# nh273/caro-ai

Hardware: NVIDIA B200
Metric: connect4_mcts_leaf_evals_per_sec (higher is better)
Workload: dtype f16

## Files before the change

caro-ai_b200/csrc/net.cu:

```cuda
#include <cuda_runtime.h>
#include <math.h>

#include <atomic>

#include "../../include/caro_b200.h"
#include "common_host.h"
#include "net.h"
#include "rules.cuh"

namespace caro {

__device__ __forceinline__ float lrelu(float x) { return x > 0.0f ? x : kLeaky * x; }

template <class R, int F>
__global__ void __launch_bounds__(256)
net_simt_kernel(R rules, const typename R::Board* __restrict__ boards, const uint8_t* __restrict__ who,
                const int32_t* __restrict__ d_count, long long max_count, const float* __restrict__ blob, BlobLayout L,
                int A, float* __restrict__ probs, float* __restrict__ values) {
  extern __shared__ float sm[];
  const int H = rules.rows(), W = rules.cols(), HW = H * W;
  const long long count = d_count ? min((long long)*d_count, max_count) : max_count;
  float* buf0 = sm;
  float* buf1 = sm + F * HW;
  for (long long leaf = blockIdx.x; leaf < count; leaf += gridDim.x) {
// ... 139 lines not shown
  if (ce != cudaSuccess) return caro_fail(CARO_E_CUDA, cudaGetErrorString(ce));
  if (net->layout.filters == kWideFilters) return caro_net_wide_pack(net, h_blob);
  const int rc = caro_net_tc_pack(net, h_blob);
  if (rc != CARO_OK) return rc;
  if (!caro_net_rt_supports(net)) return CARO_OK;
  const int rc2 = caro_net_rt_pack(net, h_blob);
  return rc2 != CARO_OK ? rc2 : caro_net_rx_pack(net, h_blob);
}

static int net_create(int rows, int cols, int actions, const BlobLayout& layout, const float* h_blob, size_t n_floats, caro_net** out) {
  static std::atomic<unsigned long long> next_serial{0};
  caro_net* net = new caro_net();
  net->serial = ++next_serial;
  net->version = 0;
  net->H = rows;
  net->W = cols;
  net->A = actions;
  net->layout = layout;
  net->d_blob = nullptr;
  net->d_tc_weights = nullptr;
  net->d_rt_weights = nullptr;
  net->d_rt_pair_weights = nullptr;
  net->d_rt_f16_weights = nullptr;
  net->d_tc_pair_weights = nullptr;
  net->d_rt_scratch = nullptr;
  net->rt_scratch_seq = 0;
  net->d_rx_weights = nullptr;
  net->d_wide_weights = nullptr;
  net->d_tc_bias = nullptr;
  net->d_pol_fc_t = nullptr;
  net->d_trace = nullptr;
  net->d_headfeat = nullptr;
  net->d_heads_b = nullptr;
  net->headfeat_leaves = 0;
  net->headfeat_seq = 0;
  net->grid_limit = 0;
  net->pipeline_limit = 0;
  {
    int dev = 0;
    cudaGetDevice(&dev);
    net->sm_count = 148;
    cudaDeviceGetAttribute(&net->sm_count, cudaDevAttrMultiProcessorCount, dev);
    int prc = caro_net_tc_prepare();
    if (prc == CARO_OK) prc = caro_net_rt_prepare();
    if (prc == CARO_OK) prc = caro_net_rx_prepare();
    if (prc == CARO_OK) prc = caro_net_heads_prepare();
// ... 113 lines not shown
```

caro-ai_b200/csrc/net.h:

```cpp
#pragma once
#include <cuda_runtime.h>
#include <stddef.h>
#include <stdint.h>

namespace caro {

constexpr int kFilters = 64;
constexpr int kWideFilters = 128;
constexpr int kBlocks = 5;
constexpr int kMaxBlocks = 20;
constexpr float kLeaky = 0.01f;

struct BlobLayout {
  size_t conv_in_w, conv_in_b;
  size_t conv_w[kMaxBlocks], conv_b[kMaxBlocks];
  int blocks;
  int filters;
  size_t val_conv_w, val_conv_b, val_fc1_w, val_fc1_b, val_fc2_w, val_fc2_b;
  size_t pol_conv_w, pol_conv_b, pol_fc_w, pol_fc_b;
  size_t total;
};

inline BlobLayout blob_layout(int H, int W, int A, int blocks = kBlocks, int filters = kFilters) {
  BlobLayout L;
// ... 15 lines not shown
  L.val_fc1_w = take(20 * hw);
  L.val_fc1_b = take(20);
  L.val_fc2_w = take(20);
  L.val_fc2_b = take(1);
  L.pol_conv_w = take(2 * F);
  L.pol_conv_b = take(2);
  L.pol_fc_w = take((size_t)A * 2 * hw);
  L.pol_fc_b = take(A);
  L.total = o;
  return L;
}

}

struct caro_net {
  int H, W, A;
  caro::BlobLayout layout;
  float* d_blob;
  void* d_tc_weights;
  void* d_rt_weights;
  void* d_tc_pair_weights;
  void* d_rt_f16_weights;
  void* d_rt_pair_weights;
  void* d_rt_scratch;
  unsigned rt_scratch_seq;
  void* d_rx_weights;
  void* d_wide_weights;
  alignas(16) float h_rt_consts[(caro::kMaxBlocks + 1) * 64 + 3 * 64 + 4 + 1536 + 4];
  float* d_tc_bias;
  float* d_pol_fc_t;
  void* d_headfeat;
  void* d_heads_b;
  long long headfeat_leaves;
  unsigned headfeat_seq;
  void* d_trace;
  int sm_count;
  int grid_limit;
  unsigned long long serial;
  unsigned long long version;
  int pipeline_limit;
};

void caro_pipeline_forget(unsigned long long engine_serial, unsigned long long net_serial);

int caro_net_tc_pack(caro_net* net, const float* h_blob);
int caro_net_tc_prepare();
// ... 31 lines not shown
```

caro-ai_b200/csrc/net_rt.cu:

```cuda
#include <cuda_bf16.h>
#include <cuda_fp16.h>
#include <cuda_fp8.h>
#include <cuda_runtime.h>
#include <math.h>
#include <string.h>

#include <type_traits>
#include <vector>

#include "../../include/caro_b200.h"
#include "common_host.h"
#include "net.h"
#include "rules.cuh"

#include "tc_common.cuh"
#include "rt_common.cuh"

#ifndef CARO_RT_MAXREG
#define CARO_RT_MAXREG 96
#endif
#ifndef CARO_RT_CP
#define CARO_RT_CP 2
#endif

namespace caro {

template <int CP, bool PAIR_ = false, bool F16_ = false>
struct RtCfg {
  static constexpr bool kPair = PAIR_;
  static constexpr bool kF16 = F16_;
  static_assert(!(PAIR_ && F16_), "the pair form exists for the bf16 mode only");
  static constexpr int kBlockBytes = PAIR_ ? kRtPairBlockBytes : kRtBlockBytes;
  static constexpr int kBlockUnits = kBlockBytes / 16;
  static constexpr int kRegionBytes = kRtRegionBlocks * kBlockBytes;
  static constexpr int kCP = CP;
  static constexpr int kCH = 64 / CP;
  static constexpr int kEpiWarps = 4 * CP;
  static constexpr int kEpiThreads = kEpiWarps * 32;
  static constexpr int kMmaWarp = kEpiWarps;
  static constexpr int kLoadWarp = kEpiWarps + 1;
  static constexpr int kHeadWarp = kEpiWarps + 2;
  static constexpr int kHeadWarps = 4;
  static constexpr int kHeadThreads = 32 * kHeadWarps;
  static constexpr int kThreads = kEpiThreads + 64 + kHeadThreads;
  static_assert(CP == 2 || CP == 4, "two or four channel parts");
  static_assert(CP == 2 || !PAIR_, "the pair form is built for two channel parts");
  static constexpr int kAct = 0;
  static constexpr int kWgt = kAct + kRtActBytes;
  static constexpr int kHeadF = kWgt + kRtRegions * kRegionBytes;
  static constexpr int kFc = kHeadF + (PAIR_ ? 0 : kRtHeadFloats * 4);
  static constexpr int kFcW = kFc + (PAIR_ ? 0 : kRtFcFloats * 4);
  static constexpr int kBars0 = kFcW;
  static constexpr int kNumBars = kRtRegions * kRtRegionBlocks + 2 * kRtRegions + 2 * kRtMaxH + 2;
  static constexpr int kFixed = kBars0 + kNumBars * 8 + 32;
// ... 43 lines not shown
                            (POS == 0 ? (uint64_t)kRtPairTop : POS == 2 ? (uint64_t)kRtPairBottom : 0ull);
        umma_bf16_pair(d_main, ad, bd, POS == 1 ? rt_idesc_pair(192) : rt_idesc_pair(128), 1u);
        if (POS == 2 && (i == 5 || i == NB - 1)) umma_commit_pair_a(i < 6 ? empty0 : empty1);
      } else {
        const uint64_t bd = (i < 6 ? rb0 + (uint64_t)(i * kUnits) : rb1 + (uint64_t)((i - 6) * kUnits)) + (POS == 0 ? 64ull : 0ull);
        if (POS == 1 && i == 0) {
          umma_bf16(d_main, ad, bd, rt_idesc_fmt<F16>(128), 1u);
          umma_bf16(d_new, ad, bd + 128ull, rt_idesc_fmt<F16>(64), 0u);
        } else {
          umma_bf16(d_main, ad, bd, POS == 1 ? rt_idesc_fmt<F16>(192) : rt_idesc_fmt<F16>(128), (POS == 0 && i == 0) ? 0u : 1u);
        }
        if (POS == 2 && (i == 5 || i == NB - 1)) umma_commit_a(i < 6 ? empty0 : empty1);
      }
    }
  }
}

template <class R, class K, int HC>
__global__ void __maxnreg__(CARO_RT_MAXREG)
net_rt_kernel(R rules, RtGeom gm, const typename R::Board* __restrict__ boards, const uint8_t* __restrict__ who,
              const int32_t* __restrict__ d_count, long long max_count, const uint8_t* __restrict__ wimg,
              const __grid_constant__ RtConsts consts, const float* __restrict__ blob, BlobLayout L,
              const float* __restrict__ pol_fc_t, const float* __restrict__ val_fc1_t, float* __restrict__ probs,
              float* __restrict__ values, long long* __restrict__ trace, float* __restrict__ scratch) {
  constexpr bool PAIR = K::kPair;
  extern __shared__ __align__(128) uint8_t smem[];
  uint8_t* act = smem + K::kAct;
  uint8_t* wgt = smem + K::kWgt;
  float* headf_s = PAIR ? scratch + (size_t)blockIdx.x * (kRtHeadFloats + kRtFcFloats) : reinterpret_cast<float*>(smem + K::kHeadF);
  float* fc_s = PAIR ? headf_s + kRtHeadFloats : reinterpret_cast<float*>(smem + K::kFc);
  uint64_t* bar_full = reinterpret_cast<uint64_t*>(smem + K::kBars);
  uint64_t* bar_empty = bar_full + kRtRegions * kRtRegionBlocks;
  uint64_t* bar_fullp = bar_empty + kRtRegions;
  uint64_t* bar_acc = bar_fullp + kRtRegions;
  uint64_t* bar_act = bar_acc + kRtMaxH;
  uint64_t* bar_feat = bar_act + kRtMaxH;
  uint32_t* tmem_slot = reinterpret_cast<uint32_t*>(bar_feat + 2);

  const int tid = threadIdx.x;
  const int warp = tid >> 5;
  if (tid == 0) TC_TRACE(7, 0);
  long long* gt_slot = nullptr;
  if (trace != nullptr && tid == 0 && (blockIdx.x == 0 || blockIdx.x == gridDim.x - 1) && trace[7998] == 2) {
    long long* base = trace + 8000 + (blockIdx.x == 0 ? 0 : 4096);
    const long long k = base[0];
    base[0] = k + 1;
    if (k < 2040) {
      gt_slot = base + 1 + 2 * k;
// ... 67 lines not shown
    }
    asm volatile("bar.sync 2, %0;" ::"n"(K::kHeadThreads) : "memory");
    for (int gi = 0; gi + 1 < my_groups; ++gi) {
      const long long leaf0 = group_leaf0(gi);
      const int nvalid = group_valid(leaf0);
      mbar_wait_relaxed(bar_feat + 0, (uint32_t)gi & 1u);
      rt_heads<K::kHeadThreads, 2>(gm, nvalid, leaf0, htid, headf_s, fc_s, consts.headb[0], consts.headb[1], consts.headb[2], fcv, polw,
                                   valw, probs, values, consts);
      mbar_arrive(bar_feat + 1);
      if (htid == 0) TC_TRACE(5, gi);
    }
    {
      const int gi = my_groups - 1;
      const long long leaf0 = group_leaf0(gi);
      const int nvalid = group_valid(leaf0);
      mbar_wait(bar_feat + 0, (uint32_t)gi & 1u);
      rt_heads<K::kEpiThreads + K::kHeadThreads, 3>(gm, nvalid, leaf0, K::kEpiThreads + htid, headf_s, fc_s, consts.headb[0],
                                                    consts.headb[1], consts.headb[2], fcv, polw, valw, probs, values, consts);
      if (htid == 0) TC_TRACE(5, gi);
    }
  } else if (warp == K::kLoadWarp) {
    if ((tid & 31) == 0) {
      const int regions_net = 2 * gm.layers - 1;
      const int total = my_groups * regions_net;
      const uint8_t* wrank = wimg + (size_t)rank * regions_net * K::kRegionBytes;
      int reg = 0, src = 0;
      uint32_t round = 0;
      for (int n = 0; n < total; ++n) {
        if (round > 0) mbar_wait_relaxed(bar_empty + reg, (round - 1u) & 1u);
        const int nblk = src == 0 ? 3 : kRtRegionBlocks;
        uint64_t* bar = bar_full + reg * kRtRegionBlocks;
        mbar_expect_tx(bar, (uint32_t)(nblk * K::kBlockBytes));
        for (int b = 0; b < nblk; ++b)
          bulk_g2s(wgt + (reg * kRtRegionBlocks + b) * K::kBlockBytes, wrank + (size_t)(src * kRtRegionBlocks + b) * K::kBlockBytes,
                   (uint32_t)K::kBlockBytes, bar);
        if (++reg == kRtRegions) { reg = 0; ++round; }
        if (++src == regions_net) src = 0;
      }
    }
  } else if (warp == K::kMmaWarp && PAIR && rank != 0) {
    if ((tid & 31) == 0) {
      const int total = my_groups * (2 * gm.layers - 1);
      const uint32_t fullp_leader = mapa_a(smem_u32(bar_fullp), 0u);
      int reg = 0;
      uint32_t ph = 0;
      for (int n = 0; n < total; ++n) {
        mbar_wait(bar_full + reg * kRtRegionBlocks, ph);
        mbar_arrive_cluster_a(fullp_leader + 8u * (uint32_t)reg);
        if (++reg == kRtRegions) { reg = 0; ph ^= 1u; }
      }
    }
  } else if (warp == K::kMmaWarp) {
    uint32_t elected;
    asm volatile("{\n\t.reg .pred P;\n\telect.sync _|P, 0xffffffff;\n\tselp.u32 %0, 1, 0, P;\n\t}" : "=r"(elected));
    const uint64_t a_desc0 = make_desc(smem_u32(act) + (uint32_t)kRtHalo * 16u, (uint32_t)kRtChunkBytes, 128u);
    const uint64_t b_desc0 = make_desc(smem_u32(wgt), (PAIR ? (uint32_t)kRtPairRows : 192u) * 16u, 128u);
    uint32_t full_a = smem_u32(bar_full), empty_a = smem_u32(bar_empty), acc_a = smem_u32(bar_acc), act_a = smem_u32(bar_act);
    uint32_t fullp_a = smem_u32(bar_fullp);
    asm volatile("" : "+r"(full_a), "+r"(empty_a), "+r"(acc_a), "+r"(act_a), "+r"(fullp_a));
    const bool tr = elected && trace != nullptr && blockIdx.x == 0;
#define RT_MMA_TRACE(kind, idx)                                                 \
  do {                                                                          \
    if (tr && (idx) < 1000) trace[(kind) * 1000 + (idx)] = clock64();           \
  } while (0)
    const int n_layers = gm.layers;
    const int total_layers = my_groups * n_layers;
    int reg = 0;
    uint32_t rphase = 0;
    int layer = 0;
    bool pre_waited = false;
    struct LayerW {
      uint64_t rb0, rb1;
      uint32_t full0, full1, empty0, empty1, ph0, ph1, fullp0, fullp1;
    };
    auto take_regions = [&](bool first_l) {
      LayerW w;
      w.rb0 = b_desc0 + (uint64_t)(uint32_t)(reg * kRtRegionBlocks * K::kBlockUnits);
      w.full0 = full_a + 8u * (uint32_t)(reg * kRtRegionBlocks);
      w.empty0 = empty_a + 8u * (uint32_t)reg;
      w.fullp0 = fullp_a + 8u * (uint32_t)reg;
      w.ph0 = rphase;
      if (++reg == kRtRegions) { reg = 0; rphase ^= 1u; }
      w.rb1 = w.rb0;
      w.full1 = w.full0;
      w.empty1 = w.empty0;
      w.fullp1 = w.fullp0;
      w.ph1 = w.ph0;
      if (!first_l) {
        w.rb1 = b_desc0 + (uint64_t)(uint32_t)(reg * kRtRegionBlocks * K::kBlockUnits);
        w.full1 = full_a + 8u * (uint32_t)(reg * kRtRegionBlocks);
        w.empty1 = empty_a + 8u * (uint32_t)reg;
        w.fullp1 = fullp_a + 8u * (uint32_t)reg;
        w.ph1 = rphase;
        if (++reg == kRtRegions) { reg = 0; rphase ^= 1u; }
      }
      return w;
    };
    LayerW nxt = take_regions(true);
    for (int gl = 0; gl < total_layers; ++gl) {
      const uint32_t par = (uint32_t)gl & 1u;
      RT_MMA_TRACE(6, gl * 2);
      const bool first = layer == 0;
      const LayerW cur = nxt;
      const uint64_t rb0 = cur.rb0, rb1 = cur.rb1;
      const uint32_t full0 = cur.full0, full1 = cur.full1, empty0 = cur.empty0, empty1 = cur.empty1, ph0 = cur.ph0, ph1 = cur.ph1;
      const uint32_t fullp0 = cur.fullp0, fullp1 = cur.fullp1;
      auto mid = [&]() {
        nxt = take_regions(layer + 1 == n_layers);
        asm volatile("" : "+l"(nxt.rb0), "+l"(nxt.rb1), "+r"(nxt.full0), "+r"(nxt.full1), "+r"(nxt.empty0), "+r"(nxt.empty1), "+r"(nxt.ph0),
                     "+r"(nxt.ph1));
        if (PAIR) asm volatile("" : "+r"(nxt.fullp0), "+r"(nxt.fullp1));
      };
      auto tile = [&](auto yv) {
        const int y = rt_value(yv);
        if (y == 0 && !pre_waited) {
          if (PAIR) {
            mbar_wait_cluster_a(act_a, par);
            mbar_wait_cluster_a(act_a + 8u, par);
          } else {
            mbar_wait_a(act_a, par);
            mbar_wait_a(act_a + 8u, par);
          }
        }
        if (y == 0) RT_MMA_TRACE(6, gl * 2 + 1);
        tc_fence_after();
        RT_MMA_TRACE(0, gl * 8 + y);
        const uint64_t a_tile = a_desc0 + (uint64_t)(uint32_t)(y * 128);
        uint64_t rb0t = rb0, rb1t = rb1;
        asm volatile("" : "+l"(rb0t), "+l"(rb1t));
        const uint32_t d_main = tmem_base + (uint32_t)(y == 0 ? 0 : (y - 1) * 64);
        const uint32_t d_new = tmem_base + (uint32_t)((y + 1) * 64);
        uint32_t nb0 = 0u, nb1 = 0u;
        uint32_t npar = par;
        if (y + 2 < H) {
          nb0 = act_a + 8u * (uint32_t)(y + 2);
        } else if (y == H - 1 && H >= 4 && gl + 1 < total_layers) {
          nb0 = act_a;
          nb1 = act_a + 8u;
          npar = par ^ 1u;
        }
        if (first) {
          if (y == 0) rt_issue_tile<0, true, PAIR, K::kF16>(y == 1, mid, elected, a_tile, rb0t, rb1t, d_main, d_new, full0, full1, ph0, ph1, empty0, empty1, nb0, nb1, npar, fullp0, fullp1);
          else if (y == H - 1) rt_issue_tile<2, true, PAIR, K::kF16>(y == 1, mid, elected, a_tile, rb0t, rb1t, d_main, d_new, full0, full1, ph0, ph1, empty0, empty1, nb0, nb1, npar, fullp0, fullp1);
          else rt_issue_tile<1, true, PAIR, K::kF16>(y == 1, mid, elected, a_tile, rb0t, rb1t, d_main, d_new, full0, full1, ph0, ph1, empty0, empty1, nb0, nb1, npar, fullp0, fullp1);
        } else {
          if (y == 0) rt_issue_tile<0, false, PAIR, K::kF16>(y == 1, mid, elected, a_tile, rb0t, rb1t, d_main, d_new, full0, full1, ph0, ph1, empty0, empty1, nb0, nb1, npar, fullp0, fullp1, tr && gl < 100 ? trace + 5000 + gl * 6 : nullptr);
          else if (y == H - 1) rt_issue_tile<2, false, PAIR, K::kF16>(y == 1, mid, elected, a_tile, rb0t, rb1t, d_main, d_new, full0, full1, ph0, ph1, empty0, empty1, nb0, nb1, npar, fullp0, fullp1);
          else rt_issue_tile<1, false, PAIR, K::kF16>(y == 1, mid, elected, a_tile, rb0t, rb1t, d_main, d_new, full0, full1, ph0, ph1, empty0, empty1, nb0, nb1, npar, fullp0, fullp1);
        }
        if (elected) {
          if (PAIR) umma_commit_pair_a(acc_a + 8u * (uint32_t)y);
          else umma_commit_a(acc_a + 8u * (uint32_t)y);
        }
        RT_MMA_TRACE(1, gl * 8 + y);
        __syncwarp();
      };
      if constexpr (HC == 6) {
        tile(RtInt<0>{});
        tile(RtInt<1>{});
        tile(RtInt<2>{});
        tile(RtInt<3>{});
        tile(RtInt<4>{});
        tile(RtInt<5>{});
      } else {
#pragma unroll 1
        for (int y = 0; y < H; ++y) tile(y);
      }
      pre_waited = H >= 4 && gl + 1 < total_layers;
      if (++layer == n_layers) layer = 0;
    }
#undef RT_MMA_TRACE
  } else {
    const int quarter = warp & 3, cp = warp >> 2;
    constexpr int CH = K::kCH, QN = CH / 4, C8N = CH / 8;
    const int row = quarter * 32 + (tid & 31);
    const int bidx = row >> gm.pshift, col = row & (gm.pitch - 1);
    const bool real = col < gm.W;
    const uint32_t lane_base = (uint32_t)(quarter * 32) << 16;
    const int HW = gm.H * gm.W;
    const bool dbg_skip_epilogue = trace != nullptr && trace[7999] == 1;
    const uint32_t act_leader = PAIR ? mapa_a(smem_u32(bar_act), 0u) : 0u;
    auto act_arrive = [&](int y) {
      if (PAIR) {
        __syncwarp();
        if ((tid & 31) == 0) mbar_arrive_cluster_a(act_leader + 8u * (uint32_t)y);
      } else {
        mbar_arrive(bar_act + y);
      }
    };
    const bool dbg_no_zero = trace != nullptr && (trace[7996] & 1);
    auto zero_acc = [&](int y, int c0) {
      if (dbg_no_zero) return;
      const uint32_t a = tmem_base + lane_base + (uint32_t)(y * 64 + c0);
      TMEM_ST16Z(a, 0u);
      TMEM_ST16Z(a + 16u, 0u);
    };

    auto write_inputs = [&](int y, long long leaf0, int writer) {
      if (cp == writer) {
        uint32_t lo = 0u;
        const long long leaf = leaf0 + bidx;
        if (real && leaf < count) {
          const typename R::Board s = boards[leaf];
          const int wm = who[leaf];
          constexpr uint32_t kOne = K::kF16 ? 0x3C00u : 0x3F80u;
          const uint32_t mine = rules.plane_value(s, wm, 0, y, col) ? kOne : 0u;
          const uint32_t other = rules.plane_value(s, wm, 1, y, col) ? kOne : 0u;
          lo = mine | (other << 16);
        }
        uint8_t* dst = act + (size_t)(kRtHalo + y * 128 + row) * 16;
        *reinterpret_cast<uint4*>(dst) = make_uint4(lo, 0u, 0u, 0u);
        *reinterpret_cast<uint4*>(dst + kRtChunkBytes) = make_uint4(0u, 0u, 0u, 0u);
        fence_async_smem();
      }
      act_arrive(y);
    };

    auto load_values = [&](auto has_res_c, int layer, int y, int c0, float2* v, uint8_t* arow) {
      constexpr bool HAS_RES = decltype(has_res_c)::value;
      const uint32_t a_acc = tmem_base + lane_base + (uint32_t)(y * 64 + c0);
      const uint32_t a_lo = tmem_base + lane_base + kRtLoCol + (uint32_t)(y * 16 + c0 / 4);
      const float4* bl4 = reinterpret_cast<const float4*>(consts.bias + layer * 64 + c0);
      uint32_t ra[CH], rl[QN];
      uint4 hv[C8N];
      TMEM_LD16(a_acc, ra);
      if (CH == 32) TMEM_LD16(a_acc + 16u, (ra + CH - 16));
      if (HAS_RES) {
        if (!K::kF16) {
          if (CH == 32) TMEM_LD8(a_lo, rl);
          else TMEM_LD4(a_lo, rl);
        }
#pragma unroll
        for (int c8 = 0; c8 < C8N; ++c8) hv[c8] = *reinterpret_cast<const uint4*>(arow + (size_t)c8 * kRtChunkBytes);
      }
      asm volatile("tcgen05.wait::ld.sync.aligned;" ::: "memory");
      const float2 slope = make_float2(kLeaky, kLeaky);
#pragma unroll
      for (int q = 0; q < QN; ++q) {
// ... 49 lines not shown
            const __nv_bfloat162 h = __floats2bfloat162_rn(vv.x, vv.y);
            const uint32_t hw = *reinterpret_cast<const uint32_t*>(&h);
            packed[j] = real ? hw : 0u;
            v[c8 * 4 + j] = __ffma2_rn(bf16x2_to_float2(hw), minus1, vv);
          }
        }
        *reinterpret_cast<uint4*>(arow + (size_t)c8 * kRtChunkBytes) = make_uint4(packed[0], packed[1], packed[2], packed[3]);
      }
      if (!K::kF16) {
        uint32_t rl[QN];
#pragma unroll
        for (int q = 0; q < QN; ++q) rl[q] = float_to_e5m2x4(v[q * 2], v[q * 2 + 1]);
        const uint32_t a_lo = tmem_base + lane_base + kRtLoCol + (uint32_t)(y * 16 + cp * QN);
        if (CH == 32) TMEM_ST8(a_lo, rl);
        else TMEM_ST4(a_lo, rl);
        asm volatile("tcgen05.wait::st.sync.aligned;" ::: "memory");
      }
      fence_async_smem();
      tc_fence_before();
      act_arrive(y);
      if (tid == 0) TC_TRACE(3, gl * 8 + y);
    };

    auto last_tile = [&](int gi, int gl, int y, bool more, long long next_leaf0) {
      mbar_wait(bar_acc + min(y + 1, H - 1), (uint32_t)gl & 1u);
      __syncwarp();
      tc_fence_after();
      if (tid == 0) TC_TRACE(2, gl * 8 + y);
      if (!dbg_skip_epilogue && (y % K::kCP) == cp) {
        float av = 0.0f, ap0 = 0.0f, ap1 = 0.0f;
#pragma unroll 1
        for (int hh = 0; hh < K::kCP; ++hh) {
          uint8_t* arow = act + (size_t)(hh * C8N * kRtActRows + kRtHalo + y * 128 + row) * 16;
          float2 v[CH / 2];
          load_values(std::true_type{}, gm.layers - 1, y, hh * CH, v, arow);
          if (PAIR) zero_acc(y, hh * CH);
          const float4* hw4 = reinterpret_cast<const float4*>(consts.headw + hh * CH);
#pragma unroll
          for (int q = 0; q < QN; ++q) {
            const float4 w0 = hw4[q], w1 = hw4[16 + q], w2 = hw4[32 + q];
            const float2 a = v[q * 2], b = v[q * 2 + 1];
            av = fmaf(a.x, w0.x, fmaf(a.y, w0.y, fmaf(b.x, w0.z, fmaf(b.y, w0.w, av))));
            ap0 = fmaf(a.x, w1.x, fmaf(a.y, w1.y, fmaf(b.x, w1.z, fmaf(b.y, w1.w, ap0))));
            ap1 = fmaf(a.x, w2.x, fmaf(a.y, w2.y, fmaf(b.x, w2.z, fmaf(b.y, w2.w, ap1))));
          }
        }
        if (real) {
          const int cell = y * gm.W + col;
          headf_s[(bidx * 3 + 0) * HW + cell] = av;
          headf_s[(bidx * 3 + 1) * HW + cell] = ap0;
          headf_s[(bidx * 3 + 2) * HW + cell] = ap1;
        }
        if (PAIR) asm volatile("tcgen05.wait::st.sync.aligned;" ::: "memory");
      }
      tc_fence_before();
      if (more) write_inputs(y, next_leaf0, y % K::kCP);
      if (tid == 0) TC_TRACE(3, gl * 8 + y);
    };

    if (PAIR) {
      for (int c = cp * 192; c < cp * 192 + 192; c += 32) zero_acc(0, c);
      asm volatile("tcgen05.wait::st.sync.aligned;" ::: "memory");
      tc_fence_before();
    }
    for (int y = 0; y < H; ++y) write_inputs(y, group_leaf0(0), 0);
    for (int gi = 0; gi < my_groups; ++gi) {
      const long long leaf0 = group_leaf0(gi);
      const bool more = gi + 1 < my_groups;
      const long long next_leaf0 = group_leaf0(gi + 1);
      const int gl0 = gi * gm.layers;
#pragma unroll 1
      for (int y = 0; y < H; ++y) epilogue_tile(std::false_type{}, 0, gl0, y);
#pragma unroll 1
      for (int layer = 1; layer < gm.layers - 1; ++layer) {
#pragma unroll 1
        for (int y = 0; y < H; ++y) epilogue_tile(std::true_type{}, layer, gl0 + layer, y);
      }
      if (gi > 0) mbar_wait(bar_feat + 1, (uint32_t)(gi - 1) & 1u);
#pragma unroll 1
      for (int y = 0; y < H; ++y) last_tile(gi, gl0 + gm.layers - 1, y, more, next_leaf0);
      mbar_arrive(bar_feat + 0);
      if (tid == 0) TC_TRACE(4, gi);
      if (!more) {
        mbar_wait(bar_feat + 0, (uint32_t)gi & 1u);
        const int nvalid = group_valid(leaf0);
        const float* fcv = reinterpret_cast<const float*>(smem + K::kFcW);
        const int fcv_floats = (41 + gm.A + 3) & ~3;
        const bool staged = fcv_floats + HW * (2 * gm.A + 20) <= K::kFcWFloats;
        const float* polw = staged ? fcv + fcv_floats : pol_fc_t;
        const float* valw = staged ? fcv + fcv_floats + 2 * HW * gm.A : val_fc1_t;
        rt_heads<K::kEpiThreads + K::kHeadThreads, 3>(gm, nvalid, leaf0, tid, headf_s, fc_s, consts.headb[0], consts.headb[1],
                                                      consts.headb[2], fcv, polw, valw, probs, values, consts);
      }
    }
  }

  if (tid == 0) TC_TRACE(7, 2);
  tc_fence_before();
  __syncthreads();
  if (PAIR) cluster_sync_all();
  if (tid == 0) TC_TRACE(7, 3);
  if (gt_slot != nullptr) {
    long long t;
    asm volatile("mov.u64 %0, %%globaltimer;" : "=l"(t));
    gt_slot[1] = t;
  }
  if (warp == K::kMmaWarp) {
    __syncwarp();
    if (PAIR) asm volatile("tcgen05.dealloc.cta_group::2.sync.aligned.b32 %0, %1;" ::"r"(tmem_base), "r"(kRtTmemCols) : "memory");
    else asm volatile("tcgen05.dealloc.cta_group::1.sync.aligned.b32 %0, %1;" ::"r"(tmem_base), "r"(kRtTmemCols) : "memory");
  }
}

static uint16_t rt_f32_to_f16(float f) {
  uint32_t u;
  memcpy(&u, &f, 4);
  const uint32_t sign = (u >> 16) & 0x8000u;
  const uint32_t absu = u & 0x7fffffffu;
  if (absu >= 0x7f800000u) return (uint16_t)(sign | (absu > 0x7f800000u ? 0x7e00u : 0x7c00u));
  if (absu >= 0x477ff000u) return (uint16_t)(sign | 0x7c00u);
  if (absu < 0x33000001u) return (uint16_t)sign;
  int e = (int)(absu >> 23) - 127;
  uint32_t m = (absu & 0x7fffffu) | 0x800000u;
  int shift = e >= -14 ? 13 : 13 + (-14 - e);
  uint32_t q = m >> shift, rem = m & ((1u << shift) - 1u), half = 1u << (shift - 1);
  if (rem > half || (rem == half && (q & 1u))) ++q;
  const uint32_t out = e >= -14 ? (((uint32_t)(e + 15) << 10) + (q - 0x400u)) : q;
  return (uint16_t)(sign | out);
}

static uint16_t rt_f32_to_bf16(float f) {
  uint32_t u;
  memcpy(&u, &f, 4);
// ... 52 lines not shown
      for (int a = 0; a < A; ++a)
        for (int i = 0; i < 2 * HW; ++i) hc->fcw[(size_t)i * A + a] = h[L.pol_fc_w + (size_t)a * 2 * HW + i];
      for (int i = 0; i < 20; ++i)
        for (int c = 0; c < HW; ++c) hc->fcw[(size_t)2 * HW * A + (size_t)c * 20 + i] = h[L.val_fc1_w + (size_t)i * HW + c];
    }
  }
  const size_t n_blocks = (size_t)(1 + 2 * blocks) * kRtRegionBlocks;
  const size_t pair_bytes = n_blocks * kRtPairBlockBytes;
  std::vector<uint16_t> pimg(2 * pair_bytes / 2, 0);
  for (int r = 0; r < 2; ++r)
    for (size_t b = 0; b < n_blocks; ++b)
      for (int chunk = 0; chunk < 2; ++chunk)
        for (int row = 0; row < kRtPairRows; ++row) {
          const int n = row < 96 ? r * 96 + row : row < 160 ? 64 + r * 64 + (row - 96) : r * 64 + (row - 160);
          const uint16_t* src = &img[(b * kRtBlockBytes + (size_t)chunk * 3072 + (size_t)n * 16) / 2];
          uint16_t* dst = &pimg[((size_t)r * pair_bytes + b * kRtPairBlockBytes + (size_t)chunk * kRtPairRows * 16 + (size_t)row * 16) / 2];
          for (int e = 0; e < 8; ++e) dst[e] = src[e];
        }
  cudaError_t ce = cudaSuccess;
  if (!net->d_rt_weights) ce = cudaMalloc(&net->d_rt_weights, img_bytes);
  if (ce == cudaSuccess) ce = cudaMemcpy(net->d_rt_weights, img.data(), img_bytes, cudaMemcpyHostToDevice);
  if (ce == cudaSuccess && !net->d_rt_f16_weights) ce = cudaMalloc(&net->d_rt_f16_weights, img_bytes);
  if (ce == cudaSuccess) ce = cudaMemcpy(net->d_rt_f16_weights, himg.data(), img_bytes, cudaMemcpyHostToDevice);
  if (ce == cudaSuccess && !net->d_rt_pair_weights) ce = cudaMalloc(&net->d_rt_pair_weights, 2 * pair_bytes);
  if (ce == cudaSuccess) ce = cudaMemcpy(net->d_rt_pair_weights, pimg.data(), 2 * pair_bytes, cudaMemcpyHostToDevice);
  if (ce == cudaSuccess && !net->d_rt_scratch)
    ce = cudaMalloc(&net->d_rt_scratch, (size_t)kRtScratchSlots * net->sm_count * (kRtHeadFloats + kRtFcFloats) * sizeof(float));
  if (ce != cudaSuccess) return caro_fail(CARO_E_CUDA, cudaGetErrorString(ce));
  return CARO_OK;
}

void caro_net_rt_free(caro_net* net) {
  if (net->d_rt_weights) cudaFree(net->d_rt_weights);
  if (net->d_rt_pair_weights) cudaFree(net->d_rt_pair_weights);
  if (net->d_rt_f16_weights) cudaFree(net->d_rt_f16_weights);
  net->d_rt_f16_weights = nullptr;
  if (net->d_rt_scratch) cudaFree(net->d_rt_scratch);
  net->d_rt_weights = nullptr;
  net->d_rt_pair_weights = nullptr;
  net->d_rt_scratch = nullptr;
}

bool caro_net_rt_supports(const caro_net* net) { return net->H >= 2 && net->H <= kRtMaxH && net->W >= 2 && net->W <= kRtMaxW; }

using RtK = RtCfg<CARO_RT_CP>;
using RtKPair = RtCfg<2, true>;
using RtKF16 = RtCfg<CARO_RT_CP, false, true>;

static bool rt_pair_enabled() {
  static const bool on = getenv("CARO_RT_PAIR") ? atoi(getenv("CARO_RT_PAIR")) != 0 : false;
  return on;
}

template <class R>
static int launch_rt(const R& rules, caro_net* net, const void* boards, const uint8_t* who, const int32_t* d_count,
                     int64_t max_count, float* probs, float* values, int mode, cudaStream_t st) {
  const bool pair = mode == 1;
  RtGeom gm;
  gm.H = net->H;
  gm.W = net->W;
  gm.A = net->A;
  gm.pshift = net->W < 4 ? 2 : 3;
  gm.pitch = 1 << gm.pshift;
  gm.nb = 128 / gm.pitch;
  gm.layers = 1 + net->layout.blocks;
  if (gm.nb * 3 * gm.H * gm.W > kRtHeadFloats || gm.nb * (20 + gm.A) > kRtFcFloats)
    return caro_fail(CARO_E_ARG, "board does not fit the row-tiled tensor-core geometry");
  const long long max_groups = (max_count + gm.nb - 1) / gm.nb;
  static const int generic_env = getenv("CARO_RT_GENERIC") ? atoi(getenv("CARO_RT_GENERIC")) : 0;
  const int lim = net->grid_limit > 0 ? net->grid_limit : net->pipeline_limit;
  const int ctas = lim > 0 && lim < net->sm_count ? lim : net->sm_count;
  if ((pair || rt_pair_enabled()) && max_groups >= 2 && ctas >= 2) {
    const long long max_units = (max_groups + 1) / 2;
    const unsigned pairs = (unsigned)(max_units < ctas / 2 ? max_units : ctas / 2);
    float* scratch = (float*)net->d_rt_scratch +
                     (size_t)(net->rt_scratch_seq++ % kRtScratchSlots) * net->sm_count * (kRtHeadFloats + kRtFcFloats);
    cudaLaunchConfig_t cfg = {};
    cfg.gridDim = dim3(2 * pairs);
    cfg.blockDim = dim3(RtKPair::kThreads);
    cfg.dynamicSmemBytes = RtKPair::kTotal;
    cfg.stream = st;
    cudaLaunchAttribute attr[1];
    attr[0].id = cudaLaunchAttributeClusterDimension;
    attr[0].val.clusterDim.x = 2;
    attr[0].val.clusterDim.y = 1;
    attr[0].val.clusterDim.z = 1;
    cfg.attrs = attr;
    cfg.numAttrs = 1;
    auto pkern = gm.H == 6 && !generic_env ? net_rt_kernel<R, RtKPair, 6> : net_rt_kernel<R, RtKPair, 0>;
    const cudaError_t ce = cudaLaunchKernelEx(
        &cfg, pkern, rules, gm, (const typename R::Board*)boards, who, d_count, (long long)max_count,
        (const uint8_t*)net->d_rt_pair_weights, *reinterpret_cast<const RtConsts*>(net->h_rt_consts), (const float*)net->d_blob, net->layout,
        (const float*)net->d_pol_fc_t, (const float*)(net->d_pol_fc_t + (size_t)2 * net->H * net->W * net->A), probs, values,
        (long long*)net->d_trace, scratch);
    if (ce != cudaSuccess) return caro_fail(CARO_E_CUDA, cudaGetErrorString(ce));
    return caro_check_launch("net_rt_kernel (pair)");
  }
  const unsigned grid = (unsigned)(max_groups < ctas ? max_groups : ctas);
  if (mode == 2) {
    auto fkern = gm.H == 6 && !generic_env ? net_rt_kernel<R, RtKF16, 6> : net_rt_kernel<R, RtKF16, 0>;
    fkern<<<grid, RtKF16::kThreads, RtKF16::kTotal, st>>>(
        rules, gm, (const typename R::Board*)boards, who, d_count, (long long)max_count, (const uint8_t*)net->d_rt_f16_weights,
        *reinterpret_cast<const RtConsts*>(net->h_rt_consts), net->d_blob, net->layout, net->d_pol_fc_t,
        net->d_pol_fc_t + (size_t)2 * net->H * net->W * net->A, probs, values, (long long*)net->d_trace, nullptr);
    return caro_check_launch("net_rt_kernel (fp16)");
  }
  auto kern = gm.H == 6 && !generic_env ? net_rt_kernel<R, RtK, 6> : net_rt_kernel<R, RtK, 0>;
  kern<<<grid, RtK::kThreads, RtK::kTotal, st>>>(
      rules, gm, (const typename R::Board*)boards, who, d_count, (long long)max_count, (const uint8_t*)net->d_rt_weights,
      *reinterpret_cast<const RtConsts*>(net->h_rt_consts), net->d_blob, net->layout, net->d_pol_fc_t, net->d_pol_fc_t + (size_t)2 * net->H * net->W * net->A, probs,
      values, (long long*)net->d_trace, nullptr);
  return caro_check_launch("net_rt_kernel");
}

int caro_net_rt_prepare() {
  cudaError_t ce = cudaSuccess;
  auto set = [&](auto kern, int bytes) {
    if (ce == cudaSuccess) ce = cudaFuncSetAttribute(kern, cudaFuncAttributeMaxDynamicSharedMemorySize, bytes);
  };
  set(net_rt_kernel<C4Rules, RtK, 0>, RtK::kTotal);
  set(net_rt_kernel<C4Rules, RtK, 6>, RtK::kTotal);
  set(net_rt_kernel<MnkRules, RtK, 0>, RtK::kTotal);
  set(net_rt_kernel<MnkRules, RtK, 6>, RtK::kTotal);
  set(net_rt_kernel<C4Rules, RtKF16, 0>, RtKF16::kTotal);
  set(net_rt_kernel<C4Rules, RtKF16, 6>, RtKF16::kTotal);
  set(net_rt_kernel<MnkRules, RtKF16, 0>, RtKF16::kTotal);
  set(net_rt_kernel<MnkRules, RtKF16, 6>, RtKF16::kTotal);
  set(net_rt_kernel<C4Rules, RtKPair, 0>, RtKPair::kTotal);
  set(net_rt_kernel<C4Rules, RtKPair, 6>, RtKPair::kTotal);
  set(net_rt_kernel<MnkRules, RtKPair, 0>, RtKPair::kTotal);
  set(net_rt_kernel<MnkRules, RtKPair, 6>, RtKPair::kTotal);
  if (ce != cudaSuccess) return caro_fail(CARO_E_CUDA, cudaGetErrorString(ce));
  return CARO_OK;
}

int caro_net_rt_forward(caro_net* net, int game, int n, int k, const void* d_boards, const uint8_t* d_who,
                        const int32_t* d_count, int64_t max_count, float* d_probs, float* d_values, int mode, cudaStream_t st) {
  if (game == CARO_GAME_CONNECT4) return launch_rt<C4Rules>(C4Rules(), net, d_boards, d_who, d_count, max_count, d_probs, d_values, mode, st);
  return launch_rt<MnkRules>(MnkRules{n, k}, net, d_boards, d_who, d_count, max_count, d_probs, d_values, mode, st);
}
```

caro-ai_b200/csrc/rules.cuh:

```cuda
#pragma once
#include <stdint.h>

#if defined(__CUDACC__)
#define CARO_HD __host__ __device__ __forceinline__
#else
#define CARO_HD inline
#endif

namespace caro {

struct Key128 {
  uint64_t lo, hi;
};

CARO_HD uint64_t mix64(uint64_t x) {
  x ^= x >> 30;
  x *= 0xbf58476d1ce4e5b9ULL;
  x ^= x >> 27;
  x *= 0x94d049bb133111ebULL;
  x ^= x >> 31;
  return x;
}

struct C4Board {
// ... 116 lines not shown
    won = won || (1 + ray(mine, r, c, -1, 1) + ray(mine, r, c, 1, -1) >= k);
    return won;
  }

  CARO_HD Key128 key(const Board& s) const {
    uint64_t a = 0x9E3779B97F4A7C15ULL, b = 0xD1B54A32D192ED03ULL;
    for (int i = 0; i < 4; ++i) {
      a = mix64(a ^ s.w[i]) + 0x632BE59BD9B4E019ULL * (uint64_t)(2 * i + 1);
      a = mix64(a ^ (s.b[i] * 0xFF51AFD7ED558CCDULL));
      b = mix64(b + s.b[i]) ^ (0xC2B2AE3D27D4EB4FULL * (uint64_t)(2 * i + 3));
      b = mix64(b + (s.w[i] ^ 0xA0761D6478BD642FULL));
    }
    return Key128{a | 1ULL, b};
  }

  CARO_HD int plane_value(const Board& s, int who, int plane, int prow, int pcol) const {
    const int idx = prow * n + pcol;
    const uint64_t* mine = who ? s.b : s.w;
    const uint64_t* other = who ? s.w : s.b;
    return test(plane == 0 ? mine : other, idx) ? 1 : 0;
  }
};

}
```

Before: 67.35 million.

## Replace first conv layer with precomputed 3x3 pattern lookup table in fp16 path

The first convolution layer (2 input planes, 3x3 kernel) is replaced by a lookup table indexed by the base-3 encoding of each cell's 3x3 neighbourhood (19683 patterns). A setup kernel runs the layer once per pattern with tensor-core MMA and stores the bias-added, leaky-ReLU fp16 outputs. At runtime the epilogue warps cp.async the matching rows into shared memory, while the MMA and load warps skip the first layer's weight regions and MMA work. This removes one layer of MMA and weight streaming per group, at the cost of gathering roughly 2.5 MB of table data through the cache and computing pattern indices.

```diff
diff --git a/caro-ai_b200/csrc/net.cu b/caro-ai_b200/csrc/net.cu
--- a/caro-ai_b200/csrc/net.cu
+++ b/caro-ai_b200/csrc/net.cu
@@ -185,6 +185,7 @@
   net->d_rt_weights = nullptr;
   net->d_rt_pair_weights = nullptr;
   net->d_rt_f16_weights = nullptr;
+  net->d_rt_conv_in_table = nullptr;
   net->d_tc_pair_weights = nullptr;
   net->d_rt_scratch = nullptr;
   net->rt_scratch_seq = 0;
diff --git a/caro-ai_b200/csrc/net.h b/caro-ai_b200/csrc/net.h
--- a/caro-ai_b200/csrc/net.h
+++ b/caro-ai_b200/csrc/net.h
@@ -61,6 +61,7 @@
   void* d_tc_pair_weights;
   void* d_rt_f16_weights;
   void* d_rt_pair_weights;
+  void* d_rt_conv_in_table;
   void* d_rt_scratch;
   unsigned rt_scratch_seq;
   void* d_rx_weights;
diff --git a/caro-ai_b200/csrc/net_rt.cu b/caro-ai_b200/csrc/net_rt.cu
--- a/caro-ai_b200/csrc/net_rt.cu
+++ b/caro-ai_b200/csrc/net_rt.cu
@@ -25,11 +25,13 @@
 
 namespace caro {
 
-template <int CP, bool PAIR_ = false, bool F16_ = false>
+template <int CP, bool PAIR_ = false, bool F16_ = false, bool TABLE_ = false>
 struct RtCfg {
   static constexpr bool kPair = PAIR_;
   static constexpr bool kF16 = F16_;
+  static constexpr bool kTable = TABLE_;
   static_assert(!(PAIR_ && F16_), "the pair form exists for the bf16 mode only");
+  static_assert(!TABLE_ || F16_, "the first-layer table holds fp16 activations");
   static constexpr int kBlockBytes = PAIR_ ? kRtPairBlockBytes : kRtBlockBytes;
   static constexpr int kBlockUnits = kBlockBytes / 16;
   static constexpr int kRegionBytes = kRtRegionBlocks * kBlockBytes;
@@ -119,8 +121,11 @@
               const int32_t* __restrict__ d_count, long long max_count, const uint8_t* __restrict__ wimg,
               const __grid_constant__ RtConsts consts, const float* __restrict__ blob, BlobLayout L,
               const float* __restrict__ pol_fc_t, const float* __restrict__ val_fc1_t, float* __restrict__ probs,
-              float* __restrict__ values, long long* __restrict__ trace, float* __restrict__ scratch) {
+              float* __restrict__ values, long long* __restrict__ trace, float* __restrict__ scratch,
+              const uint4* __restrict__ cin_table) {
   constexpr bool PAIR = K::kPair;
+  constexpr bool table = K::kTable;
+  constexpr int lay0 = table ? 1 : 0;
   extern __shared__ __align__(128) uint8_t smem[];
   uint8_t* act = smem + K::kAct;
   uint8_t* wgt = smem + K::kWgt;
@@ -234,9 +239,9 @@
   } else if (warp == K::kLoadWarp) {
     if ((tid & 31) == 0) {
       const int regions_net = 2 * gm.layers - 1;
-      const int total = my_groups * regions_net;
+      const int total = my_groups * (regions_net - lay0);
       const uint8_t* wrank = wimg + (size_t)rank * regions_net * K::kRegionBytes;
-      int reg = 0, src = 0;
+      int reg = 0, src = lay0;
       uint32_t round = 0;
       for (int n = 0; n < total; ++n) {
         if (round > 0) mbar_wait_relaxed(bar_empty + reg, (round - 1u) & 1u);
@@ -247,7 +252,7 @@
           bulk_g2s(wgt + (reg * kRtRegionBlocks + b) * K::kBlockBytes, wrank + (size_t)(src * kRtRegionBlocks + b) * K::kBlockBytes,
                    (uint32_t)K::kBlockBytes, bar);
         if (++reg == kRtRegions) { reg = 0; ++round; }
-        if (++src == regions_net) src = 0;
+        if (++src == regions_net) src = lay0;
       }
     }
   } else if (warp == K::kMmaWarp && PAIR && rank != 0) {
@@ -276,10 +281,10 @@
     if (tr && (idx) < 1000) trace[(kind) * 1000 + (idx)] = clock64();           \
   } while (0)
     const int n_layers = gm.layers;
-    const int total_layers = my_groups * n_layers;
+    const int total_layers = my_groups * (n_layers - lay0);
     int reg = 0;
     uint32_t rphase = 0;
-    int layer = 0;
+    int layer = lay0;
     bool pre_waited = false;
     struct LayerW {
       uint64_t rb0, rb1;
@@ -308,7 +313,7 @@
       }
       return w;
     };
-    LayerW nxt = take_regions(true);
+    LayerW nxt = take_regions(!table);
     for (int gl = 0; gl < total_layers; ++gl) {
       const uint32_t par = (uint32_t)gl & 1u;
       RT_MMA_TRACE(6, gl * 2);
@@ -318,7 +323,7 @@
       const uint32_t full0 = cur.full0, full1 = cur.full1, empty0 = cur.empty0, empty1 = cur.empty1, ph0 = cur.ph0, ph1 = cur.ph1;
       const uint32_t fullp0 = cur.fullp0, fullp1 = cur.fullp1;
       auto mid = [&]() {
-        nxt = take_regions(layer + 1 == n_layers);
+        nxt = take_regions(!table && layer + 1 == n_layers);
         asm volatile("" : "+l"(nxt.rb0), "+l"(nxt.rb1), "+r"(nxt.full0), "+r"(nxt.full1), "+r"(nxt.empty0), "+r"(nxt.empty1), "+r"(nxt.ph0),
                      "+r"(nxt.ph1));
         if (PAIR) asm volatile("" : "+r"(nxt.fullp0), "+r"(nxt.fullp1));
@@ -336,6 +341,7 @@
         }
         if (y == 0) RT_MMA_TRACE(6, gl * 2 + 1);
         tc_fence_after();
+        if (table && layer == 1) fence_async_smem();
         RT_MMA_TRACE(0, gl * 8 + y);
         const uint64_t a_tile = a_desc0 + (uint64_t)(uint32_t)(y * 128);
         uint64_t rb0t = rb0, rb1t = rb1;
@@ -379,7 +385,7 @@
         for (int y = 0; y < H; ++y) tile(y);
       }
       pre_waited = H >= 4 && gl + 1 < total_layers;
-      if (++layer == n_layers) layer = 0;
+      if (++layer == n_layers) layer = lay0;
     }
 #undef RT_MMA_TRACE
   } else {
@@ -426,6 +432,25 @@
         fence_async_smem();
       }
       act_arrive(y);
+    };
+
+    auto patterns = [&](long long leaf0) {
+      uint64_t pat = real ? 0ull : (uint64_t)kConvInPatterns * 0x0001000100010001ull;
+      const long long leaf = leaf0 + bidx;
+      if (real && leaf < count) {
+        const typename R::Board s = boards[leaf];
+        const int wm = who[leaf];
+#pragma unroll 1
+        for (int y = cp, j = 0; y < H; y += K::kCP, ++j) pat |= (uint64_t)conv_in_pattern(rules, s, wm, y, col) << (16 * j);
+      }
+      return pat;
+    };
+    auto table_copy = [&](int y, uint64_t pat, int c8a, int c8b) {
+      uint8_t* dst = act + (size_t)(kRtHalo + y * 128 + row) * 16;
+      const uint4* src = cin_table + ((pat >> (16 * (y / K::kCP))) & 0xffffu) * 8u;
+      for (int c8 = c8a; c8 < c8b; ++c8)
+        asm volatile("cp.async.ca.shared.global [%0], [%1], 16;" ::"r"(smem_u32(dst + (size_t)c8 * kRtChunkBytes)), "l"(src + c8)
+                     : "memory");
     };
 
     auto load_values = [&](auto has_res_c, int layer, int y, int c0, float2* v, uint8_t* arow) {
@@ -521,7 +546,7 @@
       if (tid == 0) TC_TRACE(3, gl * 8 + y);
     };
 
-    auto last_tile = [&](int gi, int gl, int y, bool more, long long next_leaf0) {
+    auto last_tile = [&](int gi, int gl, int y, bool more, long long next_leaf0, uint64_t pat) {
       mbar_wait(bar_acc + min(y + 1, H - 1), (uint32_t)gl & 1u);
       __syncwarp();
       tc_fence_after();
@@ -543,6 +568,7 @@
             ap0 = fmaf(a.x, w1.x, fmaf(a.y, w1.y, fmaf(b.x, w1.z, fmaf(b.y, w1.w, ap0))));
             ap1 = fmaf(a.x, w2.x, fmaf(a.y, w2.y, fmaf(b.x, w2.z, fmaf(b.y, w2.w, ap1))));
           }
+          if (table && more) table_copy(y, pat, hh * C8N, hh * C8N + C8N);
         }
         if (real) {
           const int cell = y * gm.W + col;
@@ -553,7 +579,14 @@
         if (PAIR) asm volatile("tcgen05.wait::st.sync.aligned;" ::: "memory");
       }
       tc_fence_before();
-      if (more) write_inputs(y, next_leaf0, y % K::kCP);
+      if (table) {
+        if (more && !dbg_skip_epilogue && (y % K::kCP) == cp)
+          asm volatile("cp.async.mbarrier.arrive.noinc.shared::cta.b64 [%0];" ::"r"(smem_u32(bar_act + y)) : "memory");
+        else if (more)
+          act_arrive(y);
+      } else if (more) {
+        write_inputs(y, next_leaf0, y % K::kCP);
+      }
       if (tid == 0) TC_TRACE(3, gl * 8 + y);
     };
 
@@ -562,14 +595,26 @@
       asm volatile("tcgen05.wait::st.sync.aligned;" ::: "memory");
       tc_fence_before();
     }
-    for (int y = 0; y < H; ++y) write_inputs(y, group_leaf0(0), 0);
+    if (table) {
+      const uint64_t pat = patterns(group_leaf0(0));
+      for (int y = cp; y < H; y += K::kCP) table_copy(y, pat, 0, C8N * K::kCP);
+      asm volatile("cp.async.wait_all;" ::: "memory");
+      fence_async_smem();
+      for (int y = 0; y < H; ++y) act_arrive(y);
+    } else {
+      for (int y = 0; y < H; ++y) write_inputs(y, group_leaf0(0), 0);
+    }
+    const int mma_layers = gm.layers - lay0;
     for (int gi = 0; gi < my_groups; ++gi) {
       const long long leaf0 = group_leaf0(gi);
       const bool more = gi + 1 < my_groups;
       const long long next_leaf0 = group_leaf0(gi + 1);
-      const int gl0 = gi * gm.layers;
+      const int gl0 = gi * mma_layers - lay0;
+      const uint64_t pat = table && more ? patterns(next_leaf0) : 0ull;
+      if (!table) {
 #pragma unroll 1
-      for (int y = 0; y < H; ++y) epilogue_tile(std::false_type{}, 0, gl0, y);
+        for (int y = 0; y < H; ++y) epilogue_tile(std::false_type{}, 0, gl0, y);
+      }
 #pragma unroll 1
       for (int layer = 1; layer < gm.layers - 1; ++layer) {
 #pragma unroll 1
@@ -577,7 +622,7 @@
       }
       if (gi > 0) mbar_wait(bar_feat + 1, (uint32_t)(gi - 1) & 1u);
 #pragma unroll 1
-      for (int y = 0; y < H; ++y) last_tile(gi, gl0 + gm.layers - 1, y, more, next_leaf0);
+      for (int y = 0; y < H; ++y) last_tile(gi, gl0 + gm.layers - 1, y, more, next_leaf0, pat);
       mbar_arrive(bar_feat + 0);
       if (tid == 0) TC_TRACE(4, gi);
       if (!more) {
@@ -608,6 +653,93 @@
     __syncwarp();
     if (PAIR) asm volatile("tcgen05.dealloc.cta_group::2.sync.aligned.b32 %0, %1;" ::"r"(tmem_base), "r"(kRtTmemCols) : "memory");
     else asm volatile("tcgen05.dealloc.cta_group::1.sync.aligned.b32 %0, %1;" ::"r"(tmem_base), "r"(kRtTmemCols) : "memory");
+  }
+}
+
+constexpr int kRtTableActBytes = 2 * kRtChunkBytes;
+constexpr int kRtTableSmem = kRtTableActBytes + 3 * kRtBlockBytes + 3 * 8 + 8;
+
+__global__ void __launch_bounds__(128) rt_conv_in_table_kernel(const uint8_t* __restrict__ wimg, const float* __restrict__ bias,
+                                                               uint4* __restrict__ table) {
+  extern __shared__ __align__(128) uint8_t smem[];
+  uint8_t* act = smem;
+  uint8_t* wgt = smem + kRtTableActBytes;
+  uint64_t* bars = reinterpret_cast<uint64_t*>(wgt + 3 * kRtBlockBytes);
+  uint32_t* tmem_slot = reinterpret_cast<uint32_t*>(bars + 3);
+  const int tid = threadIdx.x, warp = tid >> 5;
+  const int b = tid >> 2, col = tid & 3, p = blockIdx.x * 32 + b;
+  for (int i = tid; i < kRtTableActBytes / 16; i += 128) reinterpret_cast<uint4*>(act)[i] = make_uint4(0, 0, 0, 0);
+  __syncthreads();
+  if (col < 3 && p < kConvInPatterns) {
+    int p3 = 1;
+    for (int i = 0; i < col; ++i) p3 *= 3;
+    for (int y = 0; y < 3; ++y, p3 *= 27) {
+      const int st = (p / p3) % 3;
+      *reinterpret_cast<uint4*>(act + (size_t)(kRtHalo + y * 128 + tid) * 16) = make_uint4(st == 1 ? 0x3C00u : st == 2 ? 0x3C000000u : 0u, 0, 0, 0);
+    }
+  }
+  fence_async_smem();
+  if (tid == 0) {
+    for (int i = 0; i < 3; ++i) mbar_init(bars + i, 1);
+    asm volatile("fence.mbarrier_init.release.cluster;" ::: "memory");
+  }
+  if (warp == 0) {
+    __syncwarp();
+    asm volatile("tcgen05.alloc.cta_group::1.sync.aligned.shared::cta.b32 [%0], %1;" ::"r"(smem_u32(tmem_slot)), "r"(256) : "memory");
+    asm volatile("tcgen05.relinquish_alloc_permit.cta_group::1.sync.aligned;" ::: "memory");
+  }
+  tc_fence_before();
+  __syncthreads();
+  tc_fence_after();
+  const uint32_t tmem_base = *tmem_slot;
+  if (warp == 0) {
+    if (tid == 0) {
+      mbar_expect_tx(bars, 3 * kRtBlockBytes);
+      for (int i = 0; i < 3; ++i) bulk_g2s(wgt + i * kRtBlockBytes, wimg + (size_t)i * kRtBlockBytes, kRtBlockBytes, bars);
+    }
+    uint32_t elected;
+    asm volatile("{\n\t.reg .pred P;\n\telect.sync _|P, 0xffffffff;\n\tselp.u32 %0, 1, 0, P;\n\t}" : "=r"(elected));
+    const uint64_t a0 = make_desc(smem_u32(act) + (uint32_t)kRtHalo * 16u, (uint32_t)kRtChunkBytes, 128u);
+    const uint64_t rb = make_desc(smem_u32(wgt), 192u * 16u, 128u);
+    const uint32_t full = smem_u32(bars), empty = full + 8u, acc = full + 16u;
+    auto none = [] {};
+    tc_fence_after();
+    rt_issue_tile<0, true, false, true>(false, none, elected, a0, rb, rb, tmem_base, tmem_base + 64u, full, full, 0u, 0u, empty, empty, 0u, 0u, 0u, 0u, 0u);
+    rt_issue_tile<1, true, false, true>(false, none, elected, a0 + 128u, rb, rb, tmem_base, tmem_base + 128u, full, full, 0u, 0u, empty, empty, 0u, 0u, 0u, 0u, 0u);
+    rt_issue_tile<2, true, false, true>(false, none, elected, a0 + 256u, rb, rb, tmem_base + 64u, tmem_base + 192u, full, full, 0u, 0u, empty, empty, 0u, 0u, 0u, 0u, 0u);
+    if (elected) umma_commit_a(acc);
+    __syncwarp();
+  }
+  mbar_wait(bars + 2, 0u);
+  tc_fence_after();
+  const uint32_t a_acc = tmem_base + ((uint32_t)(warp * 32) << 16) + 64u;
+  uint32_t ra[64];
+  TMEM_LD16(a_acc, ra);
+  TMEM_LD16(a_acc + 16u, (ra + 16));
+  TMEM_LD16(a_acc + 32u, (ra + 32));
+  TMEM_LD16(a_acc + 48u, (ra + 48));
+  asm volatile("tcgen05.wait::ld.sync.aligned;" ::: "memory");
+  if (col == 1 && p < kConvInPatterns) {
+    const float2 slope = make_float2(kLeaky, kLeaky);
+#pragma unroll
+    for (int c8 = 0; c8 < 8; ++c8) {
+      uint32_t packed[4];
+#pragma unroll
+      for (int j = 0; j < 4; ++j) {
+        const int c = c8 * 8 + j * 2;
+        const float2 x = __fadd2_rn(make_float2(__uint_as_float(ra[c]), __uint_as_float(ra[c + 1])), make_float2(bias[c], bias[c + 1]));
+        const float2 t = __fmul2_rn(x, slope);
+        const __half2 h = __floats2half2_rn(fmaxf(x.x, t.x), fmaxf(x.y, t.y));
+        packed[j] = *reinterpret_cast<const uint32_t*>(&h);
+      }
+      table[(size_t)p * 8 + c8] = make_uint4(packed[0], packed[1], packed[2], packed[3]);
+    }
+  }
+  tc_fence_before();
+  __syncthreads();
+  if (warp == 0) {
+    __syncwarp();
+    asm volatile("tcgen05.dealloc.cta_group::1.sync.aligned.b32 %0, %1;" ::"r"(tmem_base), "r"(256) : "memory");
   }
 }
 
@@ -706,6 +838,16 @@
   if (ce == cudaSuccess) ce = cudaMemcpy(net->d_rt_weights, img.data(), img_bytes, cudaMemcpyHostToDevice);
   if (ce == cudaSuccess && !net->d_rt_f16_weights) ce = cudaMalloc(&net->d_rt_f16_weights, img_bytes);
   if (ce == cudaSuccess) ce = cudaMemcpy(net->d_rt_f16_weights, himg.data(), img_bytes, cudaMemcpyHostToDevice);
+  if (ce == cudaSuccess && !net->d_rt_conv_in_table) {
+    ce = cudaMalloc(&net->d_rt_conv_in_table, (size_t)(kConvInPatterns + 1) * 128);
+    if (ce == cudaSuccess) ce = cudaMemset((uint8_t*)net->d_rt_conv_in_table + (size_t)kConvInPatterns * 128, 0, 128);
+  }
+  if (ce == cudaSuccess) {
+    rt_conv_in_table_kernel<<<(kConvInPatterns + 31) / 32, 128, kRtTableSmem>>>(
+        (const uint8_t*)net->d_rt_f16_weights, net->d_blob + L.conv_in_b, (uint4*)net->d_rt_conv_in_table);
+    ce = cudaGetLastError();
+    if (ce == cudaSuccess) ce = cudaDeviceSynchronize();
+  }
   if (ce == cudaSuccess && !net->d_rt_pair_weights) ce = cudaMalloc(&net->d_rt_pair_weights, 2 * pair_bytes);
   if (ce == cudaSuccess) ce = cudaMemcpy(net->d_rt_pair_weights, pimg.data(), 2 * pair_bytes, cudaMemcpyHostToDevice);
   if (ce == cudaSuccess && !net->d_rt_scratch)
@@ -719,6 +861,8 @@
   if (net->d_rt_pair_weights) cudaFree(net->d_rt_pair_weights);
   if (net->d_rt_f16_weights) cudaFree(net->d_rt_f16_weights);
   net->d_rt_f16_weights = nullptr;
+  if (net->d_rt_conv_in_table) cudaFree(net->d_rt_conv_in_table);
+  net->d_rt_conv_in_table = nullptr;
   if (net->d_rt_scratch) cudaFree(net->d_rt_scratch);
   net->d_rt_weights = nullptr;
   net->d_rt_pair_weights = nullptr;
@@ -729,7 +873,8 @@
 
 using RtK = RtCfg<CARO_RT_CP>;
 using RtKPair = RtCfg<2, true>;
-using RtKF16 = RtCfg<CARO_RT_CP, false, true>;
+using RtKF16 = RtCfg<CARO_RT_CP, false, true, true>;
+using RtKF16Mma = RtCfg<CARO_RT_CP, false, true, false>;
 
 static bool rt_pair_enabled() {
   static const bool on = getenv("CARO_RT_PAIR") ? atoi(getenv("CARO_RT_PAIR")) != 0 : false;
@@ -776,24 +921,29 @@
         &cfg, pkern, rules, gm, (const typename R::Board*)boards, who, d_count, (long long)max_count,
         (const uint8_t*)net->d_rt_pair_weights, *reinterpret_cast<const RtConsts*>(net->h_rt_consts), (const float*)net->d_blob, net->layout,
         (const float*)net->d_pol_fc_t, (const float*)(net->d_pol_fc_t + (size_t)2 * net->H * net->W * net->A), probs, values,
-        (long long*)net->d_trace, scratch);
+        (long long*)net->d_trace, scratch, (const uint4*)nullptr);
     if (ce != cudaSuccess) return caro_fail(CARO_E_CUDA, cudaGetErrorString(ce));
     return caro_check_launch("net_rt_kernel (pair)");
   }
   const unsigned grid = (unsigned)(max_groups < ctas ? max_groups : ctas);
   if (mode == 2) {
-    auto fkern = gm.H == 6 && !generic_env ? net_rt_kernel<R, RtKF16, 6> : net_rt_kernel<R, RtKF16, 0>;
+    const char* cin_env = getenv("CARO_RT_CONV_IN_MMA");
+    const bool mma = cin_env && atoi(cin_env) != 0;
+    const uint4* cin_table = (const uint4*)net->d_rt_conv_in_table;
+    auto fkern = mma ? (gm.H == 6 && !generic_env ? net_rt_kernel<R, RtKF16Mma, 6> : net_rt_kernel<R, RtKF16Mma, 0>)
+                     : (gm.H == 6 && !generic_env ? net_rt_kernel<R, RtKF16, 6> : net_rt_kernel<R, RtKF16, 0>);
+    static_assert(RtKF16Mma::kTotal == RtKF16::kTotal && RtKF16Mma::kThreads == RtKF16::kThreads, "one launch shape for both forms");
     fkern<<<grid, RtKF16::kThreads, RtKF16::kTotal, st>>>(
         rules, gm, (const typename R::Board*)boards, who, d_count, (long long)max_count, (const uint8_t*)net->d_rt_f16_weights,
         *reinterpret_cast<const RtConsts*>(net->h_rt_consts), net->d_blob, net->layout, net->d_pol_fc_t,
-        net->d_pol_fc_t + (size_t)2 * net->H * net->W * net->A, probs, values, (long long*)net->d_trace, nullptr);
+        net->d_pol_fc_t + (size_t)2 * net->H * net->W * net->A, probs, values, (long long*)net->d_trace, nullptr, cin_table);
     return caro_check_launch("net_rt_kernel (fp16)");
   }
   auto kern = gm.H == 6 && !generic_env ? net_rt_kernel<R, RtK, 6> : net_rt_kernel<R, RtK, 0>;
   kern<<<grid, RtK::kThreads, RtK::kTotal, st>>>(
       rules, gm, (const typename R::Board*)boards, who, d_count, (long long)max_count, (const uint8_t*)net->d_rt_weights,
       *reinterpret_cast<const RtConsts*>(net->h_rt_consts), net->d_blob, net->layout, net->d_pol_fc_t, net->d_pol_fc_t + (size_t)2 * net->H * net->W * net->A, probs,
-      values, (long long*)net->d_trace, nullptr);
+      values, (long long*)net->d_trace, nullptr, nullptr);
   return caro_check_launch("net_rt_kernel");
 }
 
@@ -810,6 +960,10 @@
   set(net_rt_kernel<C4Rules, RtKF16, 6>, RtKF16::kTotal);
   set(net_rt_kernel<MnkRules, RtKF16, 0>, RtKF16::kTotal);
   set(net_rt_kernel<MnkRules, RtKF16, 6>, RtKF16::kTotal);
+  set(net_rt_kernel<C4Rules, RtKF16Mma, 0>, RtKF16Mma::kTotal);
+  set(net_rt_kernel<C4Rules, RtKF16Mma, 6>, RtKF16Mma::kTotal);
+  set(net_rt_kernel<MnkRules, RtKF16Mma, 0>, RtKF16Mma::kTotal);
+  set(net_rt_kernel<MnkRules, RtKF16Mma, 6>, RtKF16Mma::kTotal);
   set(net_rt_kernel<C4Rules, RtKPair, 0>, RtKPair::kTotal);
   set(net_rt_kernel<C4Rules, RtKPair, 6>, RtKPair::kTotal);
   set(net_rt_kernel<MnkRules, RtKPair, 0>, RtKPair::kTotal);
diff --git a/caro-ai_b200/csrc/rules.cuh b/caro-ai_b200/csrc/rules.cuh
--- a/caro-ai_b200/csrc/rules.cuh
+++ b/caro-ai_b200/csrc/rules.cuh
@@ -162,4 +162,20 @@
   }
 };
 
+constexpr int kConvInPatterns = 19683;
+
+template <class R>
+CARO_HD int conv_in_pattern(const R& rules, const typename R::Board& s, int who, int y, int x) {
+  int idx = 0, p3 = 1;
+#if defined(__CUDA_ARCH__)
+#pragma unroll
+#endif
+  for (int k = 0; k < 9; ++k, p3 *= 3) {
+    const int yy = y + k / 3 - 1, xx = x + k % 3 - 1;
+    if (yy < 0 || yy >= rules.rows() || xx < 0 || xx >= rules.cols()) continue;
+    idx += rules.plane_value(s, who, 0, yy, xx) ? p3 : rules.plane_value(s, who, 1, yy, xx) ? 2 * p3 : 0;
+  }
+  return idx;
 }
+
+}
```

Result: faster. 68.22 million (median of 6 runs) (+1.3%).
